# leftfield-geospatial/homonim

Measured on AMD Instinct MI355X. Metric: Mpixels*bands/s fit+apply (5x5 gain-offset, float32), higher is better.
Workload: dtype f32 in/out, f64 window sums; 1 GPU; synthetic float32 4-band 16384x16384 src/ref resident in HBM per GPU, Model.gain-offset, kernel 5x5, r2_inpaint_thresh 0.25, fused fit+apply (BASELINE.json configs[2]); bands=4, height=16384, width=16384, nodata_variant=0, parallelism=1 rank(s) x 1 GPU, one raster per rank, no collective

## Files before the change

### homonim_amd/csrc/hk_api.hip

```cpp
#include <hip/hip_runtime.h>

#include <algorithm>
#include <atomic>
#include <cfloat>
#include <cctype>
#include <cmath>
#include <condition_variable>
#include <cstdarg>
#include <cstdio>
#include <cstdlib>
#include <cstring>
#include <map>
#include <mutex>
#include <new>
#include <optional>
#include <vector>

#include "../../include/homonim_hk.h"
#include "../../include/homonim_hk_devtools.h"
#include "hk_kernels.h"

#include <dlfcn.h>
#include <hsa/hsa.h>
#include <hsa/hsa_ext_amd.h>
// ... 204 lines not shown
    size_t norm_ws_bytes = 0;
    void* aux = nullptr;
    size_t aux_bytes = 0;
    double* comm_xchg = nullptr;
    size_t comm_xchg_bytes = 0;
    unsigned long long* fail_host = nullptr;
    static constexpr size_t PIN_NORM = 64, PIN_SUMS = 128, PIN_NORM_IN = 192, PIN_WORD = 256, PIN_STATS = 512, PIN_COUNTS = 1024, PIN_BYTES = 16384;
    template <class T> T* pin(size_t off) const { return reinterpret_cast<T*>(reinterpret_cast<char*>(fail_host) + off); }
    static constexpr int STAGE_N = 4;
    struct StageOut {
        char* h_dst = nullptr;
        size_t h_pitch = 0, row_bytes = 0, c_pitch = 0;
        size_t rows = 0;
    };
    char* stage = nullptr;
    size_t stage_chunk = 0;
    hipEvent_t stage_ev[STAGE_N] = {nullptr, nullptr, nullptr, nullptr};
    int stage_state[STAGE_N] = {0, 0, 0, 0};
    StageOut stage_out[STAGE_N];
    int stage_next = 0;
    static constexpr int TBL_RING = 4;
    void* tbl_host[TBL_RING] = {nullptr, nullptr, nullptr, nullptr};
    void* tbl_dev[TBL_RING] = {nullptr, nullptr, nullptr, nullptr};
    size_t tbl_bytes[TBL_RING] = {0, 0, 0, 0};
    hipEvent_t tbl_ev[TBL_RING] = {nullptr, nullptr, nullptr, nullptr};
    int tbl_next = 0;
    unsigned* open_rows = nullptr;
    size_t open_rows_bytes = 0;
    bool direct_pending = false;
    bool busy = false;
    int dev_inflight = 0;
    bool dev_touched = false;
};

constexpr int64_t ROW_ALIGN = 64;

struct LaunchPolicy {
    int xcd_remap = 16;
    int force_general = 0;
    std::optional<int> use_ring;
    int wave_slots = 256 * 12;
    std::optional<int> seg_big, seg_tail;
};

}

struct hk_ctx {
    int device = 0;
    std::vector<Slot> slots;
    std::mutex mu;
    std::condition_variable cv;
    LaunchPolicy launch;
    std::atomic<int> expect_r2_failures{0};
    ncclComm_t comm = nullptr;
    int comm_rank = 0, comm_world = 0;
    std::mutex comm_mu;
    Slot xfer;
    std::mutex xfer_mu;
};

struct hk_event {
    hipEvent_t ev;
};

namespace {

void stage_abandon(Slot& s);

struct SlotLease {
    hk_ctx* ctx;
    int idx;
    SlotLease(hk_ctx* c) : ctx(c), idx(-1) {
        bool drain = false;
        {
            std::unique_lock<std::mutex> lk(ctx->mu);
            ctx->cv.wait(lk, [&] {
                int any = -1;
                for (size_t i = 0; i < ctx->slots.size(); ++i) {
                    if (ctx->slots[i].busy || ctx->slots[i].dev_inflight > 0) continue;
                    if (!ctx->slots[i].dev_touched) {
                        idx = (int)i;
                        return true;
                    }
                    if (any < 0) any = (int)i;
                }
                idx = any;
                return any >= 0;
            });
            ctx->slots[idx].busy = true;
            drain = ctx->slots[idx].dev_touched;
            ctx->slots[idx].dev_touched = false;
        }
        if (drain) (void)hipStreamSynchronize(ctx->slots[idx].stream);
    }
    ~SlotLease() {
        stage_abandon(ctx->slots[idx]);
        {
            std::lock_guard<std::mutex> lk(ctx->mu);
            ctx->slots[idx].busy = false;
        }
        ctx->cv.notify_all();
    }
    Slot& slot() { return ctx->slots[idx]; }
};

struct DevEnter {
// ... 469 lines not shown
    a.seg_rows = uniform < a.height ? uniform : a.height;
    a.seg_rows_tail = a.seg_rows;
    a.n_segs = (a.height + a.seg_rows - 1) / a.seg_rows;
    a.n_segs_big = a.n_segs;
    const long long per_row_band = (long long)a.n_strips * a.n_bands;
    if (seg_rows <= 0 && per_row_band * a.n_segs >= seg.two_size_from) {
        const int big = seg.big, tail = seg.tail;
        long long tail_rows = (long long)(seg.tail_waves / (double)per_row_band * big);
        tail_rows = (tail_rows + tail - 1) / tail * tail;
        if (big > 0 && tail > 0 && tail_rows < a.height - big) {
            const int n_big = (int)((a.height - tail_rows) / big);
            const int rest = a.height - n_big * big;
            a.seg_rows = big;
            a.seg_rows_tail = tail;
            a.n_segs_big = n_big;
            a.n_segs = n_big + (rest + tail - 1) / tail;
        }
    }
    a.total_units = a.n_strips * a.n_segs * a.n_bands;
    if (a.lds_pad < 0) a.lds_pad = lds_pad_of((long long)a.height * a.width * a.n_bands);
}

static int ensure_inpaint_scratch(Slot& sl, size_t plane, int height, long long stride) {
    return grow_slot_buf(sl, sl.aux, sl.aux_bytes, plane + hk::inpaint_workspace_bytes(height, stride));
}

static bool cert_list_eligible(const hk::FitArgs& a, const hk_fit_desc* desc) {
    return desc->model == HK_MODEL_GAIN_OFFSET && a.has_thresh && a.fail_count && !a.r2 && !a.gain && !a.flag && !a.offset_in &&
           !a.jobs && (a.use_ring == 1 || a.use_ring == 2) && (long long)desc->kh * desc->kw <= 65535;
}

static int launch_fit(hk_ctx* ctx, Slot& sl, hk::FitArgs& a, const hk_fit_desc* desc, bool r2) {
    a.cert_only = 0, a.open_rows = nullptr, a.list_mode = 0;
    if (!cert_list_eligible(a, desc)) {
        HK_HIP(hk::launch_fit_apply(a, desc->model, r2, sl.stream));
        return HK_OK;
    }
    const size_t bytes = (size_t)a.n_bands * (size_t)a.n_strips * (size_t)((a.height + 31) / 32) * sizeof(unsigned);
    {
        std::lock_guard<std::mutex> lk(ctx->mu);
        const int rc = grow_slot_buf(sl, sl.open_rows, sl.open_rows_bytes, bytes);
        if (rc) return rc;
    }
    hk::FitArgs c = a;
    c.open_rows = sl.open_rows;
    HK_HIP(hipMemsetAsync(c.open_rows, 0, bytes, sl.stream));
    c.cert_only = 1;
    HK_HIP(hk::launch_fit_apply(c, desc->model, r2, sl.stream));
    c.cert_only = 0, c.list_mode = 1;
    HK_HIP(hk::launch_fit_apply(c, desc->model, r2, sl.stream));
    return HK_OK;
}

static int inpaint_band(Slot& sl, const hk::FitArgs& a, const hk_fit_desc* desc, bool r2, size_t plane,
                        unsigned long long n_fail, bool drop_params = false, float* pre_offset = nullptr,
                        const unsigned char* pre_flag = nullptr) {
    {
        const int rc = ensure_inpaint_scratch(sl, plane, a.height, a.stride);
        if (rc) return rc;
    }
    const hipStream_t stream = sl.stream;
    char* aux = static_cast<char*>(sl.aux);
    const float *pg = a.gain, *pr = a.r2;
    float* po = a.offset;
    const unsigned char* flags = nullptr;
    if (pre_offset && pre_flag) {
        po = pre_offset, flags = pre_flag;
    } else if (!pg || !po || !pr) {
        float* scratch_off = reinterpret_cast<float*>(aux);
        hk::FitArgs b = a;
        b.gain = nullptr, b.r2 = nullptr, b.offset = scratch_off, b.corr = nullptr, b.fail_count = nullptr;
        b.flag = hk::inpaint_flag_plane(aux + plane, a.height, a.stride);
        b.cert_only = 0, b.open_rows = nullptr, b.list_mode = 0;
        HK_HIP(hk::launch_fit_apply(b, desc->model, r2, stream));
        po = scratch_off, flags = b.flag;
    }
    HK_HIP(hk::launch_inpaint_offsets(po, pg, pr, desc->r2_thresh, a.stride, a.height, a.width, aux + plane, stream, flags, n_fail));
    hk::FitArgs c = a;
    c.offset_in = po;
    c.flag_in = flags ? flags : hk::inpaint_flag_plane(aux + plane, a.height, a.stride);
    c.fail_count = nullptr;
    c.flag = nullptr;
    c.r2 = nullptr;
    c.cert_only = 0, c.open_rows = nullptr, c.list_mode = 0;
    if (drop_params) c.gain = c.offset = nullptr;
    HK_HIP(hk::launch_fit_apply(c, desc->model, false, stream));
    return HK_OK;
}

int job_fit_args(hk::FitArgs& a, const hk_ctx* ctx, const hk_fit_desc* desc, const hk_dev_job& job, int band = -1) {
    const int b = band < 0 ? 0 : band;
    const long long off = (long long)b * job.band_stride;
    auto plane = [off](float* p) { return p ? p + off : nullptr; };
    memset(&a, 0, sizeof(a));
    a.src = job.src + off, a.ref = job.ref + off;
    a.gain = plane(job.gain), a.offset = plane(job.offset), a.r2 = plane(job.r2), a.corr = plane(job.corr);
    a.norm = job.norm ? job.norm + 2 * b : nullptr;
    a.fail_count = job.fail_count ? reinterpret_cast<unsigned long long*>(job.fail_count) + b : nullptr;
    a.height = job.height, a.width = job.width, a.stride = job.stride;
    a.band_stride = band < 0 ? job.band_stride : 0;
    a.n_bands = band < 0 ? job.n_bands : 1;
    fill_args(a, desc, ctx->launch);
    fill_grid(a, job.seg_rows, ctx->launch);
    if (job.out_rows || job.out_cols) {
        if (a.has_thresh)
            return fail(HK_ERR_UNSUPPORTED, "a store window is not supported together with r2_inpaint_thresh (the in-painting "
                                            "needs the parameters of the whole block)");
        a.out_y0 = job.out_row0, a.out_y1 = job.out_row0 + job.out_rows;
        a.out_x0 = job.out_col0, a.out_x1 = job.out_col0 + job.out_cols;
    }
    return HK_OK;
}

hk::NormArgs norm_args(const hk_fit_desc* desc, const float* src, const float* ref, int height, int width, long long stride,
                       long long band_stride = 0, int n_bands = 1) {
    hk::NormArgs na;
    na.src = src, na.ref = ref, na.height = height, na.width = width, na.stride = stride;
    na.band_stride = band_stride, na.n_bands = n_bands;
    na.src_nd_mode = desc->src_nodata_mode, na.ref_nd_mode = desc->ref_nodata_mode;
    na.src_nodata = desc->src_nodata, na.ref_nodata = desc->ref_nodata;
    return na;
}

struct FitPending {
    hk::FitArgs a;
    bool scratch_params = false;
    bool active = false;
};

int fit_finish(hk_ctx* ctx, Slot& sl, const hk_fit_desc* desc, FitPending& p, unsigned long long n_fail, bool* requeued) {
    *requeued = false;
    if (!p.active) return HK_OK;
    hk::FitArgs& a = p.a;
    const bool r2 = needs_r2(desc);
    const size_t plane = (size_t)a.stride * a.height * sizeof(float);
    ctx->expect_r2_failures.store(n_fail > 0 ? 1 : 0);
    if (n_fail > 0) {
        const int rc = inpaint_band(sl, a, desc, r2, plane, n_fail, p.scratch_params, a.flag ? a.offset : nullptr, a.flag);
        if (rc) return rc;
        *requeued = true;
    }
    return HK_OK;
}

int fit_on_device(hk_ctx* ctx, Slot& sl, const hk_fit_desc* desc, const double* norm_in, float* d_src, float* d_ref,
                  int32_t height, int32_t width, int64_t stride, float* d_gain, float* d_off, float* d_r2, float* d_corr,
                  double* d_norm, unsigned long long* d_fail, void* d_norm_ws, FitPending* defer = nullptr,
                  const int* win = nullptr) {
    const bool blk = desc->model == HK_MODEL_GAIN_BLK_OFFSET;
    const bool r2 = needs_r2(desc);
    const size_t plane = (size_t)stride * height * sizeof(float);
    HK_HIP(hipMemsetAsync(d_fail, 0, sizeof(unsigned long long), sl.stream));
    if (blk) {
        if (norm_in) {
            memcpy(sl.pin<double>(Slot::PIN_NORM_IN), norm_in, 2 * sizeof(double));
            HK_HIP(hipMemcpyAsync(d_norm, sl.pin<double>(Slot::PIN_NORM_IN), 2 * sizeof(double), hipMemcpyHostToDevice, sl.stream));
        } else {
            HK_HIP(hk::launch_block_norm(norm_args(desc, d_src, d_ref, height, width, stride), d_norm_ws, d_norm, sl.stream));
        }
    }
    hk_dev_job job = {};
    job.src = d_src, job.ref = d_ref, job.gain = d_gain, job.offset = d_off, job.r2 = d_r2, job.corr = d_corr;
    job.norm = blk ? d_norm : nullptr;
    job.fail_count = reinterpret_cast<uint64_t*>(d_fail);
    job.n_bands = 1, job.height = height, job.width = width, job.stride = stride;
    if (win && !(desc->model == HK_MODEL_GAIN_OFFSET && desc->has_r2_thresh))
        job.out_row0 = win[0], job.out_rows = win[1] - win[0], job.out_col0 = win[2], job.out_cols = win[3] - win[2];
    FitPending local;
    FitPending& p = defer ? *defer : local;
    hk::FitArgs& a = p.a;
    int rc = job_fit_args(a, ctx, desc, job);
    if (rc) return rc;
    p.scratch_params = false;
    if (a.has_thresh && desc->model == HK_MODEL_GAIN_OFFSET && ctx->expect_r2_failures.load()) {
        rc = ensure_inpaint_scratch(sl, plane, height, stride);
        if (rc) return rc;
        char* aux = static_cast<char*>(sl.aux);
        a.flag = hk::inpaint_flag_plane(aux + plane, height, stride);
        if (!d_off) {
            a.offset = reinterpret_cast<float*>(aux);
            p.scratch_params = !d_gain && !d_r2;
        }
    }
    rc = launch_fit(ctx, sl, a, desc, r2);
    if (rc) return rc;
    p.active = a.has_thresh != 0;
    if (defer || !p.active) return HK_OK;

    HK_HIP(hipMemcpyAsync(sl.fail_host, d_fail, sizeof(unsigned long long), hipMemcpyDeviceToHost, sl.stream));
    HK_HIP(hipStreamSynchronize(sl.stream));
    bool requeued = false;
// ... 170 lines not shown
    int n = 0;
    if (hipGetDeviceCount(&n) != hipSuccess || n < 1)
        return fail(HK_ERR_NODEVICE, "no HIP device available (libhomonim_hk needs an MI355X / gfx950 GPU)");
    if (device_id < 0 || device_id >= n) return fail(HK_ERR_ARG, "device %d out of range [0, %d)", device_id, n);
    if (n_streams < 1) n_streams = 1;
    if (n_streams > 64) n_streams = 64;
    HK_HIP(hipSetDevice(device_id));
    hipDeviceProp_t prop;
    HK_HIP(hipGetDeviceProperties(&prop, device_id));
    if (strncmp(prop.gcnArchName, "gfx950", 6) != 0)
        return fail(HK_ERR_NODEVICE, "device %d is %s; this library is built for gfx950 only", device_id, prop.gcnArchName);
    hk_ctx* ctx = new (std::nothrow) hk_ctx();
    if (!ctx) return fail(HK_ERR_NOMEM, "out of host memory");
    ctx->device = device_id;
    ctx->slots.resize(n_streams);
    {
        auto env = [](const char* name) { const char* e = getenv(name); return e ? std::optional<int>(atoi(e)) : std::nullopt; };
        LaunchPolicy& lp = ctx->launch;
        if (const auto remap = env("HK_XCD_REMAP")) lp.xcd_remap = std::min(std::max(*remap, 0), 256);
        lp.force_general = env("HK_FORCE_GENERAL").value_or(0);
        lp.use_ring = env("HK_USE_RING");
        lp.wave_slots = env("HK_WAVE_SLOTS").value_or(lp.wave_slots);
        lp.seg_big = env("HK_SEG_BIG");
        lp.seg_tail = env("HK_SEG_TAIL");
    }
    for (auto& s : ctx->slots) {
        hipError_t e = hipStreamCreateWithFlags(&s.stream, hipStreamNonBlocking);
        if (e != hipSuccess) {
            hk_ctx_destroy(ctx);
            return fail(HK_ERR_HIP, "hipStreamCreate: %s", hipGetErrorString(e));
        }
        if (ensure_pin(s) != HK_OK) {
            hk_ctx_destroy(ctx);
            return HK_ERR_NOMEM;
        }
    }
    {
        hipError_t e = hipStreamCreateWithFlags(&ctx->xfer.stream, hipStreamNonBlocking);
        if (e != hipSuccess || ensure_pin(ctx->xfer) != HK_OK) {
            hk_ctx_destroy(ctx);
            return e != hipSuccess ? fail(HK_ERR_HIP, "hipStreamCreate: %s", hipGetErrorString(e)) : HK_ERR_NOMEM;
        }
    }
    register_gpu_fault_report();
    *out = ctx;
    return HK_OK;
}

int hk_ctx_destroy(hk_ctx* ctx) {
    if (!ctx) return HK_OK;
    (void)hipSetDevice(ctx->device);
    for (auto& s : ctx->slots) slot_release(s);
    slot_release(ctx->xfer);
    if (ctx->comm && rccl().ok) rccl().CommDestroy(ctx->comm);
    delete ctx;
    return HK_OK;
}

int hk_ctx_sync(hk_ctx* ctx) {
    if (!ctx) return fail(HK_ERR_ARG, "ctx is NULL");
    HK_ENTER(ctx);
    HK_HIP(hipDeviceSynchronize());
    return HK_OK;
}

int hk_block_norm(hk_ctx* ctx, const hk_fit_desc* desc, const float* src, int64_t src_stride, const float* ref,
                  int64_t ref_stride, int32_t height, int32_t width, double norm_out[2]) {
    if (!norm_out) return fail(HK_ERR_ARG, "norm_out is NULL");
    return run_host(ctx, desc, nullptr, src, src_stride, ref, ref_stride, height, width, nullptr, nullptr, 0, nullptr,
                    norm_out, nullptr, true);
}

int hk_fit(hk_ctx* ctx, const hk_fit_desc* desc, const float* src, int64_t src_stride, const float* ref,
           int64_t ref_stride, int32_t height, int32_t width, const double* norm_in, float* params_out,
           int32_t n_param_bands, double* norm_out, uint64_t* r2_fail_count) {
    if (!params_out) return fail(HK_ERR_ARG, "params_out is NULL");
    return run_host(ctx, desc, nullptr, src, src_stride, ref, ref_stride, height, width, norm_in, params_out,
                    n_param_bands, nullptr, norm_out, r2_fail_count, false);
}

int hk_fit_apply(hk_ctx* ctx, const hk_fit_desc* desc, const float* src, int64_t src_stride, const float* ref,
                 int64_t ref_stride, int32_t height, int32_t width, const double* norm_in, float* params_out,
                 int32_t n_param_bands, float* corr_out, double* norm_out, uint64_t* r2_fail_count) {
    if (!corr_out) return fail(HK_ERR_ARG, "corr_out is NULL");
    return run_host(ctx, desc, nullptr, src, src_stride, ref, ref_stride, height, width, norm_in, params_out,
                    n_param_bands, corr_out, norm_out, r2_fail_count, false);
}

int hk_fit_apply_io(hk_ctx* ctx, const hk_fit_desc* desc, const hk_io_desc* io, const void* src, int64_t src_stride,
                    const void* ref, int64_t ref_stride, int32_t height, int32_t width, const double* norm_in,
                    float* params_out, int32_t n_param_bands, void* corr_out, double* norm_out, uint64_t* r2_fail_count) {
    return run_host(ctx, desc, io, src, src_stride, ref, ref_stride, height, width, norm_in, params_out, n_param_bands,
                    corr_out, norm_out, r2_fail_count, false);
}

int hk_fit_apply_block(hk_ctx* ctx, const hk_fit_desc* desc, const hk_io_desc* io, const void* src, int64_t src_stride,
                       const void* ref, int64_t ref_stride, int32_t height, int32_t width, const double* norm_in,
                       float* params_out, int32_t n_param_bands, void* corr_out, const hk_out_window* window,
                       double* norm_out, uint64_t* r2_fail_count) {
    return run_host(ctx, desc, io, src, src_stride, ref, ref_stride, height, width, norm_in, params_out, n_param_bands,
                    corr_out, norm_out, r2_fail_count, false, window);
}

int hk_apply(hk_ctx* ctx, const float* src, int64_t src_stride, const float* params, int32_t height, int32_t width,
             float* out) {
    if (!ctx) return fail(HK_ERR_ARG, "ctx is NULL");
// ... 529 lines not shown
    HK_HIP(hipMemcpyAsync(host_counts, job->fail_count, bytes, hipMemcpyDeviceToHost, sl.stream));
    HK_HIP(hipMemsetAsync(job->fail_count, 0, bytes, sl.stream));
    HK_HIP(hipEventRecord(ready->ev, sl.stream));
    return HK_OK;
}

int hk_debug_stage_stamps(hk_ctx* ctx, uint64_t out[16], int32_t reset) {
    if (!ctx || !out) return fail(HK_ERR_ARG, "NULL argument");
    HK_ENTER(ctx);
    HK_HIP(hipDeviceSynchronize());
    unsigned long long tmp[16];
    HK_HIP(hk::read_stamps(tmp, reset != 0));
    for (int i = 0; i < 16; ++i) out[i] = tmp[i];
    return HK_OK;
}

int hk_r2_certificate_constants(float thresh, double* pass_below, double* fail_above, float* kappa, float* kappa_fail) {
    if (pass_below) *pass_below = r2_pass_scale(thresh);
    if (fail_above) *fail_above = r2_fail_above(thresh);
    if (kappa) *kappa = r2_fail_scale(thresh);
    if (kappa_fail) *kappa_fail = r2_failcert_scale(thresh);
    return HK_OK;
}

int hk_counts_pending(const uint64_t* counts, int32_t n_bands) {
    if (!counts) return 0;
    for (int32_t b = 0; b < n_bands; ++b)
        if (counts[b]) return 1;
    return 0;
}

int hk_event_sync(hk_ctx* ctx, hk_event* ev) {
    if (!ctx || !ev) return fail(HK_ERR_ARG, "NULL argument");
    HK_ENTER(ctx);
    HK_HIP(hipEventSynchronize(ev->ev));
    return HK_OK;
}

int hk_inpaint_dev_counts(hk_ctx* ctx, const hk_fit_desc* desc, const hk_dev_job* job, const uint64_t* counts,
                          uint64_t* n_fail_out) {
    int rc = validate_desc(desc);
    if (rc) return rc;
    rc = check_job(ctx, job);
    if (rc) return rc;
    DevEnter entered(ctx, job->stream);
    if (n_fail_out) *n_fail_out = 0;
    if (desc->model != HK_MODEL_GAIN_OFFSET || !desc->has_r2_thresh) return HK_OK;
    if (!counts) return fail(HK_ERR_ARG, "counts is NULL");
    HK_ENTER(ctx);
    Slot& sl = ctx->slots[job->stream];
    const bool r2 = needs_r2(desc);
    const size_t plane = (size_t)job->stride * job->height * sizeof(float);
    unsigned long long total = 0;
    for (int b = 0; b < job->n_bands; ++b) {
        unsigned long long n_fail = counts[b];
        if (n_fail == 0) continue;
        const long long off = (long long)b * job->band_stride;
        hk::FitArgs a;
        if ((rc = job_fit_args(a, ctx, desc, *job, b))) return rc;
        std::unique_lock<std::mutex> lk(ctx->mu);
        float* pre_off = nullptr;
        const unsigned char* pre_flag = nullptr;
        if (job->scratch) {
            pre_flag = job_scratch_flag(job) + off;
            pre_off = a.offset ? a.offset : job_scratch_offset(job) + off;
        }
        total += n_fail;
        rc = inpaint_band(sl, a, desc, r2, plane, n_fail, false, pre_off, pre_flag);
        if (rc) return rc;
    }
    if (n_fail_out) *n_fail_out = total;
    return HK_OK;
}

int hk_inpaint_dev(hk_ctx* ctx, const hk_fit_desc* desc, const hk_dev_job* job, uint64_t* n_fail_out) {
    int rc = validate_desc(desc);
    if (rc) return rc;
    rc = check_job(ctx, job);
    if (rc) return rc;
    DevEnter entered(ctx, job->stream);
    if (n_fail_out) *n_fail_out = 0;
    if (desc->model != HK_MODEL_GAIN_OFFSET || !desc->has_r2_thresh) return HK_OK;
    if (!job->fail_count) return fail(HK_ERR_ARG, "job->fail_count is NULL");
    if (job->n_bands > 1024) return fail(HK_ERR_ARG, "too many bands");
    HK_ENTER(ctx);
    Slot& sl = ctx->slots[job->stream];
    std::vector<uint64_t> counts((size_t)job->n_bands);
    uint64_t* const pinned = sl.pin<uint64_t>(Slot::PIN_COUNTS);
    HK_HIP(hipMemcpyAsync(pinned, job->fail_count, counts.size() * sizeof(uint64_t), hipMemcpyDeviceToHost, sl.stream));
    HK_HIP(hipStreamSynchronize(sl.stream));
    memcpy(counts.data(), pinned, counts.size() * sizeof(uint64_t));
    HK_HIP(hipMemsetAsync(job->fail_count, 0, counts.size() * sizeof(uint64_t), sl.stream));
    return hk_inpaint_dev_counts(ctx, desc, job, counts.data(), n_fail_out);
}

static int ensure_stream_ws(hk_ctx* ctx, Slot& sl, size_t need) {
    std::lock_guard<std::mutex> lk(ctx->mu);
    return grow_slot_buf(sl, sl.norm_ws, sl.norm_ws_bytes, need);
}

static int check_nodata_mode(int32_t mode) {
    return (mode == HK_NODATA_NONE || mode == HK_NODATA_NAN || mode == HK_NODATA_VALUE)
               ? HK_OK
               : fail(HK_ERR_ARG, "bad nodata mode %d", mode);
}

int hk_compare_sums_dev(hk_ctx* ctx, const hk_dev_job* job, int32_t src_nodata_mode, float src_nodata,
                        int32_t ref_nodata_mode, float ref_nodata, double* sums_dev) {
    int rc = check_job(ctx, job);
    if (rc) return rc;
    DevEnter entered(ctx, job->stream);
    if (!sums_dev) return fail(HK_ERR_ARG, "sums_dev is NULL");
    if ((rc = check_nodata_mode(src_nodata_mode)) || (rc = check_nodata_mode(ref_nodata_mode))) return rc;
    HK_ENTER(ctx);
    Slot& sl = ctx->slots[job->stream];
    rc = ensure_stream_ws(ctx, sl, hk::compare_workspace_bytes(job->n_bands));
    if (rc) return rc;
    hk::CompareArgs ca;
    memset(&ca, 0, sizeof(ca));
    ca.src = job->src, ca.ref = job->ref, ca.height = job->height, ca.width = job->width;
    ca.src_stride = ca.ref_stride = job->stride, ca.src_band_stride = ca.ref_band_stride = job->band_stride;
// ... 614 lines not shown
```

### homonim_amd/csrc/hk_fit_kernel.h

```cpp
#pragma once
#include "hk_kernels.h"

#include <type_traits>

namespace hk {

static __device__ unsigned long long hk_stamps[16];
#ifdef HK_STAMPS
#define HK_STAMP(k)                                                       \
    do {                                                                  \
        __builtin_amdgcn_sched_barrier(0);                                \
        const unsigned long long now_ = __builtin_amdgcn_s_memtime();     \
        st_acc[k] += now_ - st_prev;                                      \
        st_prev = now_;                                                   \
        __builtin_amdgcn_sched_barrier(0);                                \
    } while (0)
#else
#define HK_STAMP(k) do { } while (0)
#endif
static inline hipError_t read_stamps_tu(unsigned long long* acc16, bool reset) {
    unsigned long long v[16];
    hipError_t e = hipMemcpyFromSymbol(v, HIP_SYMBOL(hk_stamps), sizeof(v));
    if (e != hipSuccess) return e;
    for (int k = 0; k < 16; ++k) acc16[k] += v[k];
// ... 1219 lines not shown
                                } else if constexpr (BLK) {
                                    q = __dmul_rn((double)__fmul_rn(gp[i], gp[i]), HS2[i]);
                                    q = __dsub_rn(q, __dmul_rn((double)__fmul_rn(2.f, gp[i]), HP[i]));
                                    q = __dadd_rn(q, HR2[i]);
                                } else {
                                    q = __dmul_rn((double)__fmul_rn(g[i], g[i]), HS2[i]);
                                    q = __dsub_rn(q, (double)__fmul_rn(__fmul_rn(2.f, g[i]), Pf[i]));
                                    q = __dadd_rn(q, HR2[i]);
                                }
                                ssres[i] = __dmul_rn(q, (double)Nf[i]);
                            }
                            bool r2_ok[PX];
                            bool divide = !GO || a.r2 != nullptr;
                            if constexpr (GO) {
                                if (!divide) {
                                    bool unsure = false;
#pragma unroll
                                    for (int i = 0; i < PX; ++i) {
                                        const bool pos = sstot[i] > 0.0;
                                        const bool yes = pos & (ssres[i] < __dmul_rn(a.r2_pass_below, sstot[i]));
                                        const bool no = pos & (ssres[i] > __dmul_rn(a.r2_fail_above, sstot[i]));
                                        r2_ok[i] = yes;
                                        unsure |= out_lane & (bool)((mcu >> (8 * i)) & 1u) & !(yes | no);
                                    }
                                    divide = __any(unsure);
                                }
                            }
#pragma unroll
                            for (int i = 0; i < PX; ++i) {
                                if (divide) {
                                    r2v[i] = __fsub_rn(1.f, (float)__ddiv_rn(ssres[i], sstot[i]));
                                    r2_ok[i] = r2v[i] > a.r2_thresh;
                                }
                                if constexpr (GO) {
                                    const bool m = (mcu >> (8 * i)) & 1u;
                                    if (!(r2_ok[i] && (g[i] > 0.f))) passed &= ~(0xffu << (8 * i));
                                    const bool failing = count_fails && m && !(r2_ok[i] && (g[i] > 0.f));
                                    if (failing && out_lane) ++nfail;
                                    if (failing && inpaint_pass && out_lane) {
                                        const float oin = a.offset_in[out_base + (long long)y * a.stride + x + i];
                                        o[i] = oin;
                                        g[i] = __fdiv_rn(__fsub_rn(Rf[i], __fmul_rn(Nf[i], oin)), Sf[i]);
                                    }
                                }
                            }
                        }
                    }
                }

                if constexpr (GO && !R2) {
                    if (a.offset_in != nullptr) {
                        const long long q = out_base + (long long)y * a.stride + (lane_in ? x : 0);
                        const float4 oin4 = *reinterpret_cast<const float4*>(a.offset_in + q);
                        const unsigned fl = *reinterpret_cast<const unsigned*>(a.flag_in + q);
                        const float oin[PX] = {oin4.x, oin4.y, oin4.z, oin4.w};
#pragma unroll
                        for (int i = 0; i < PX; ++i) {
                            const bool failing = ((mcu >> (8 * i)) & 1u) && !((fl >> (8 * i)) & 0xffu);
                            if (failing) {
                                o[i] = oin[i];
                                g[i] = __fdiv_rn(__fsub_rn(Rf[i], __fmul_rn(Nf[i], oin[i])), Sf[i]);
                            }
                        }
                    }
                }

#pragma unroll
                for (int j = 0; j < PX / 2; ++j) {
                    const f2 c2 = HK_P2(g, j) * HK_P2(sc, j) + HK_P2(o, j);
                    c[2 * j] = c2.x, c[2 * j + 1] = c2.y;
                }
                if constexpr (!DENSE) {
#pragma unroll
                    for (int i = 0; i < PX; ++i) c[i] = ((mcu >> (8 * i)) & 1u) ? c[i] : qnan();
                }
                auto masked4 = [&](const float (&v)[PX]) {
                    float4 r4 = make_float4(v[0], v[1], v[2], v[3]);
                    if constexpr (!DENSE) {
                        r4.x = (mcu & 0x00000001u) ? r4.x : qnan();
                        r4.y = (mcu & 0x00000100u) ? r4.y : qnan();
                        r4.z = (mcu & 0x00010000u) ? r4.z : qnan();
                        r4.w = (mcu & 0x01000000u) ? r4.w : qnan();
                    }
                    return r4;
                };

                if (out_lane) {
                    const long long row_off = out_base + (long long)y * a.stride;
                    auto at = [&](float* plane) {
                        if constexpr (SB) return row_address(plane + row_off) + xbytes;
                        else return reinterpret_cast<float4*>(reinterpret_cast<char*>(plane + row_off) + xbytes);
                    };
                    if (a.corr && !((HK_ABLATE & 8) && c[0] != 123.456f)) store4_nt(at(a.corr), make_float4(c[0], c[1], c[2], c[3]));
                    if constexpr (!CERT_ONLY) {
                        if (a.gain) store4_nt(at(a.gain), masked4(g));
                    }
                    if (a.offset) store4_nt(at(a.offset), masked4(o));
                    if constexpr (!CERT_ONLY) {
                        if (R2 && a.r2) store4_nt(at(a.r2), masked4(r2v));
                    }
                    if constexpr (GO && R2 && !CERT_ONLY) {
                        if (a.flag) *reinterpret_cast<unsigned*>(a.flag + row_off + (xbytes >> 2)) = passed | ((~mcu & 0x01010101u) << 1);
                    }
                }
            };
            bool skip_row = false;
            if constexpr (LIST)
                skip_row = ((a.open_rows[(size_t)(band * a.n_strips + strip) * (size_t)((H + 31) >> 5) + (size_t)(y >> 5)] >> (y & 31)) & 1u) == 0u;
            if (skip_row) {
            } else if constexpr (UNIFORM_N) {
                if (n_uniform) pointwise(std::true_type{});
                else pointwise(std::false_type{});
            } else {
                pointwise(std::false_type{});
            }
            HK_STAMP(4);
        }

        if (++slot == ring_mod) slot = 0;
        if (++slot_c == ring_mod) slot_c = 0;
        if (++slot2 == rh + 1) slot2 = 0;
        if (++slot_r >= rh) slot_r = 0;
    }
#ifdef HK_STAMPS
    if (lane == 0) {
        for (int k = 0; k < 6; ++k) atomicAdd(&hk_stamps[k], st_acc[k]);
        atomicAdd(&hk_stamps[15], st_iters);
        atomicAdd(&hk_stamps[14], 1ull);
    }
#endif

    if constexpr (GO && R2) {
        if (a.fail_count != nullptr && a.has_thresh) {
#pragma unroll
            for (int d = WAVE / 2; d > 0; d >>= 1) nfail += __shfl_xor(nfail, d);
            if (lane == 0 && nfail) atomicAdd(a.fail_count + band, (unsigned long long)nfail);

        }
    }
}

template <int MODEL, bool R2, int RW, bool DENSE, int RING, bool CERT_ONLY, int WPB, bool BATCH = false>
__global__ void __launch_bounds__(WAVE * WPB, (fit_min_waves<MODEL, R2, RW, DENSE, RING, CERT_ONLY>()))
fit_apply_kernel(const FitArgs a_in) {
    extern __shared__ float4 lds4[];

    const int lane = threadIdx.x & (WAVE - 1), wave_in_wg = (WPB == 1 && fit_scalar_bases<MODEL, R2, RW, DENSE, RING, CERT_ONLY>()) ? 0 : threadIdx.x >> 6;
    int group = blockIdx.x;
    if (a_in.xcd_remap) {
        const int g = a_in.xcd_remap / WPB > 0 ? a_in.xcd_remap / WPB : 1, slot = blockIdx.x >> 3;
        group = ((slot / g) * 8 + (blockIdx.x & 7)) * g + slot % g;
    }
    [[maybe_unused]] FitArgs a_job;
    if constexpr (BATCH) {
        constexpr int FG = WPB > 1 ? 1 : 0;
// ... 242 lines not shown
```

### homonim_amd/csrc/hk_inpaint.hip

```cpp
#include "hk_kernels.h"

#include <stdlib.h>

#define HK_SQ(v) __mul24((v), (v))

#include <type_traits>

namespace hk {


__global__ void __launch_bounds__(256) inpaint_flag_kernel(const float* __restrict__ gain, const float* __restrict__ r2,
                                                           float thresh, long long stride, int height, int width,
                                                           unsigned char* __restrict__ flag) {
    const int x = blockIdx.x * blockDim.x + threadIdx.x;
    if (x >= width) return;
    for (int y = blockIdx.y; y < height; y += gridDim.y) {
        const long long i = (long long)y * stride + x;
        flag[i] = ((r2[i] > thresh) && (gain[i] > 0.f)) ? 1 : 0;
    }
}

constexpr unsigned NONE_B = 0xffu;
constexpr unsigned NONE_SQ = 0x7fffu;
constexpr int WORD_ROWS = 64;

__global__ void __launch_bounds__(256) inpaint_bits_kernel(const unsigned char* __restrict__ flag, long long stride, int height,
                                                           int width, unsigned long long* __restrict__ bits,
                                                           unsigned long long* __restrict__ tbits) {
    const int x = (blockIdx.x * blockDim.x + threadIdx.x) * 4;
    if (x >= width) return;
    const int y0 = blockIdx.y * WORD_ROWS;
    unsigned lo[4] = {0, 0, 0, 0}, hi[4] = {0, 0, 0, 0}, tlo[4] = {0, 0, 0, 0}, thi[4] = {0, 0, 0, 0};
#pragma unroll
    for (int r = 0; r < 32; ++r) {
        const int ya = y0 + r, yb = y0 + 32 + r;
        const unsigned fa = *reinterpret_cast<const unsigned*>(flag + (long long)min(ya, height - 1) * stride + x);
        const unsigned fb = *reinterpret_cast<const unsigned*>(flag + (long long)min(yb, height - 1) * stride + x);
#pragma unroll
        for (int c = 0; c < 4; ++c) {
            lo[c] |= (unsigned)(((fa >> (8 * c)) & 1u) != 0 && ya < height) << r;
            hi[c] |= (unsigned)(((fb >> (8 * c)) & 1u) != 0 && yb < height) << r;
            tlo[c] |= (unsigned)(((fa >> (8 * c)) & 0xffu) == 0 && ya < height) << r;
            thi[c] |= (unsigned)(((fb >> (8 * c)) & 0xffu) == 0 && yb < height) << r;
        }
    }
#pragma unroll
    for (int c = 0; c < 4; ++c)
        if (x + c < width) {
            bits[(long long)blockIdx.y * stride + x + c] = ((unsigned long long)hi[c] << 32) | lo[c];
            tbits[(long long)blockIdx.y * stride + x + c] = ((unsigned long long)thi[c] << 32) | tlo[c];
        }
}

__global__ void __launch_bounds__(256) inpaint_table_kernel(const unsigned long long* __restrict__ bits, long long stride,
                                                            int height, int width, int max_dist,
                                                            unsigned* __restrict__ tb) {
    const int x = (blockIdx.x * blockDim.x + threadIdx.x) * 2;
    if (x >= width) return;
    const int wb = blockIdx.y, n_words = (height + WORD_ROWS - 1) / WORD_ROWS;
    const int y0 = wb * WORD_ROWS, rows = min(WORD_ROWS, height - y0);
    unsigned long long wm2[2], wm1[2], w0[2], wp1[2], wp2[2];
#pragma unroll
    for (int c = 0; c < 2; ++c) {
        auto word = [&](int w) { return (w >= 0 && w < n_words) ? bits[(long long)w * stride + x + c] : 0ull; };
        wm2[c] = word(wb - 2), wm1[c] = word(wb - 1), w0[c] = word(wb), wp1[c] = word(wb + 1), wp2[c] = word(wb + 2);
    }
    constexpr int BIG = 1 << 20;
    unsigned upk[2][WORD_ROWS / 4];
    int dseed[2];
#pragma unroll
    for (int c = 0; c < 2; ++c) {
        int u = wm1[c] ? __clzll((long long)wm1[c]) : (wm2[c] ? 64 + __clzll((long long)wm2[c]) : BIG);
#pragma unroll
        for (int q = 0; q < WORD_ROWS / 4; ++q) {
            unsigned pk = 0;
#pragma unroll
            for (int k = 0; k < 4; ++k) {
                const int bb = 4 * q + k;
                u = ((w0[c] >> bb) & 1ull) ? 0 : min(u + 1, BIG);
                pk |= (unsigned)(u <= max_dist ? u : (int)NONE_B) << (8 * k);
            }
            upk[c][q] = pk;
        }
        dseed[c] = wp1[c] ? 1 + (__ffsll((long long)wp1[c]) - 1) : (wp2[c] ? 65 + (__ffsll((long long)wp2[c]) - 1) : BIG);
    }
    int d[2] = {dseed[0], dseed[1]};
#pragma unroll
    for (int bb = WORD_ROWS - 1; bb >= 0; --bb) {
        unsigned e[2];
#pragma unroll
        for (int c = 0; c < 2; ++c) {
            if (bb < WORD_ROWS - 1) d[c] = ((w0[c] >> (bb + 1)) & 1ull) ? 1 : min(d[c] + 1, BIG);
            const unsigned ub = (upk[c][bb >> 2] >> (8 * (bb & 3))) & 0xffu;
            const unsigned usq = ub == NONE_B ? NONE_SQ : (unsigned)HK_SQ((int)ub);
            const unsigned dsq = d[c] <= max_dist + 1 ? (unsigned)HK_SQ(d[c]) : NONE_SQ;
            e[c] = (dsq << 16) | usq;
// ... 326 lines not shown
                (unsigned char)(slow_rows[wv][lane >> 2] >> (8 * (lane & 3)));
    }
}

#ifndef HK_FILL_TILE_WAVES
#define HK_FILL_TILE_WAVES 8
#endif
template <int ROWS>
__global__ void __launch_bounds__(256, (ROWS <= 32 ? HK_FILL_TILE_WAVES : 5))
inpaint_fill_general_kernel(float* plane, const unsigned long long* __restrict__ bits, long long stride, int height, int width,
                            const unsigned* __restrict__ tb, const unsigned* __restrict__ tie, const double* __restrict__ wtab) {
    static_assert(ROWS == 16 || ROWS == 32 || ROWS == 64, "tiles divide the 64-row words of the bit planes");
    __shared__ unsigned short lst[256 / WAVE][ROWS * WAVE];
    const int tid = threadIdx.x, lane = tid & (WAVE - 1), wv = tid / WAVE;
    const int x0 = blockIdx.x * blockDim.x + wv * WAVE, x_own = x0 + lane;
    const unsigned long long lt = (1ull << lane) - 1ull;
    const int max_dist = FILL_MAX_DIST;
    const bool interior = x0 - max_dist - 12 >= 0 && x0 + WAVE - 1 + max_dist + 12 < width;
    const int n_tiles = (height + ROWS - 1) / ROWS;
    for (int tile_k = blockIdx.y; tile_k < n_tiles; tile_k += gridDim.y) {
        const int y0 = (n_tiles - 1 - tile_k) * ROWS;
        unsigned long long tgt_rows = 0ull;
        if (x_own < width) {
            tgt_rows = bits[(long long)(y0 / WORD_ROWS) * stride + x_own] >> (y0 % WORD_ROWS);
            const int rows_in = min(ROWS, height - y0);
            tgt_rows &= rows_in >= 64 ? ~0ull : (1ull << rows_in) - 1ull;
        }
        if (__ballot(tgt_rows != 0ull) == 0ull) continue;
        int n = 0;
#pragma unroll 4
        for (int r = 0; r < ROWS; ++r) {
            const bool target = (tgt_rows >> r) & 1ull;
            const unsigned long long bal = __ballot(target);
            if (target) lst[wv][n + (int)__popcll(bal & lt)] = (unsigned short)((r << 6) | lane);
            n += (int)__popcll(bal);
        }
        __builtin_amdgcn_fence(__ATOMIC_ACQ_REL, "wavefront");
        for (int p = 0; p < n; p += WAVE) {
            if (p + lane < n) {
                const unsigned e = lst[wv][p + lane];
                const int x = x0 + (int)(e & 63u), y = y0 + (int)(e >> 6);
                const long long row = (long long)y * stride;
                const bool last_row = y == height - 1;
                const float v = interior ? fill_one<true>(x, y, row, plane, stride, width, max_dist, tb, tie, wtab, last_row)
                                         : fill_one<false>(x, y, row, plane, stride, width, max_dist, tb, tie, wtab, last_row);
                plane[row + x] = v;
            }
        }
    }
}

static size_t bit_words(int height, long long stride) { return (size_t)((height + WORD_ROWS - 1) / WORD_ROWS) * (size_t)stride; }
size_t inpaint_workspace_bytes(int height, long long stride) {
    return (size_t)height * stride * 5 + 1024 + TIE_N / 8 + 256 + WTAB_N * 8 + 256 + 3 * (bit_words(height, stride) * 8 + 256)
           + sizeof(FastTables) + 256;
}

unsigned char* inpaint_flag_plane(void* workspace, int height, long long stride) {
    return reinterpret_cast<unsigned char*>(static_cast<unsigned short*>(workspace) + 2 * (size_t)height * stride);
}

hipError_t launch_inpaint_offsets(float* offset, const float* gain, const float* r2, float thresh, long long stride,
                                  int height, int width, void* workspace, hipStream_t stream,
                                  const unsigned char* flag_ready, unsigned long long n_targets) {
    const size_t plane = (size_t)height * stride;
    unsigned* tb = static_cast<unsigned*>(workspace);
    unsigned char* ws_flag = inpaint_flag_plane(workspace, height, stride);
    const unsigned char* flag = flag_ready ? flag_ready : ws_flag;
    unsigned* tie = reinterpret_cast<unsigned*>(ws_flag + (plane + 255) / 256 * 256);
    double* wtab = reinterpret_cast<double*>(tie + (TIE_N / 32 + 64) / 64 * 64);
    HK_LAUNCH(tie_kernel, dim3((TIE_N / 32 + 255) / 256), dim3(256), 0, stream, tie, wtab);
    const int max_dist = FILL_MAX_DIST;
    static_assert(100 + 1 < (int)NONE_B, "the table's distance bytes");
    if (!flag_ready)
        HK_LAUNCH(inpaint_flag_kernel, dim3((width + 255) / 256, height < 1024 ? height : 1024), dim3(256), 0, stream,
                           gain, r2, thresh, stride, height, width, ws_flag);
    auto align256 = [](void* p) { return reinterpret_cast<void*>((reinterpret_cast<uintptr_t>(p) + 255) / 256 * 256); };
    unsigned long long* bits = static_cast<unsigned long long*>(align256(wtab + WTAB_N));
    unsigned long long* tbits = static_cast<unsigned long long*>(align256(bits + bit_words(height, stride)));
    unsigned long long* sbits = static_cast<unsigned long long*>(align256(tbits + bit_words(height, stride)));
    FastTables* ftab = static_cast<FastTables*>(align256(sbits + bit_words(height, stride)));
    HK_LAUNCH(fast_table_kernel, dim3((FTAB_N + 7 + 255) / 256), dim3(256), 0, stream, ftab);
    const dim3 gbits((width + 1023) / 1024, (height + WORD_ROWS - 1) / WORD_ROWS);
    HK_LAUNCH(inpaint_bits_kernel, gbits, dim3(256), 0, stream, flag, stride, height, width, bits, tbits);
    const dim3 gtable((width + 511) / 512, (height + WORD_ROWS - 1) / WORD_ROWS);
    HK_LAUNCH(inpaint_table_kernel, gtable, dim3(256), 0, stream, bits, stride, height, width, max_dist, tb);
    const bool by_column = (double)n_targets > 0.6 * (double)height * (double)width;
    const bool fast = stride < (1ll << 23);
    if (fast) {
        const int n_tiles8 = (height + 7) / 8, wgs_y = (n_tiles8 + 3) / 4;
        const dim3 gf((width + 255) / 256, wgs_y < 65535 ? wgs_y : 65535);
        if (by_column)
            HK_LAUNCH(inpaint_fill_fast_kernel<true>, gf, dim3(256), 0, stream, offset, tbits, sbits, stride, height, width, tb, ftab, 1);
        else
            HK_LAUNCH(inpaint_fill_fast_kernel<false>, gf, dim3(256), 0, stream, offset, tbits, sbits, stride, height, width, tb, ftab, 1);
    }
    const unsigned long long* todo = fast ? sbits : tbits;
    const int n_tiles = (height + 31) / 32;
    const dim3 gt((width + 255) / 256, n_tiles < 65535 ? n_tiles : 65535);
    HK_LAUNCH(inpaint_fill_general_kernel<32>, gt, dim3(256), 0, stream, offset, todo, stride, height, width, tb, tie, wtab);
    return hipGetLastError();
}

}
```

### homonim_amd/csrc/hk_kernels.h

```cpp
#pragma once
#include <hip/hip_runtime.h>
#include <stdint.h>
#include <string.h>

struct hk_warp_desc;

namespace hk {

constexpr int PX = 4;
constexpr int WAVE = 64;

struct BuildRecord {
    char name[88];
    unsigned long long launches;
    BuildRecord* next;
    explicit BuildRecord(const char* kernel_name);
    BuildRecord(int model, bool r2, int rw, bool dense, int ring, bool cert_only, int wpb, bool batch);
    BuildRecord(const char* kernel_name, int model, bool r2, int rw, bool dense, int ring);
    void hit() { __atomic_fetch_add(&launches, 1ull, __ATOMIC_RELAXED); }
};
template <typename Tag>
struct SiteRecord {
    static BuildRecord rec;
};
// ... 151 lines not shown
    int src_nd_mode, ref_nd_mode;
    float src_nodata, ref_nodata;
    int vec_ok;
};
size_t compare_workspace_bytes(int n_bands);
hipError_t launch_compare_sums(const CompareArgs& a, void* workspace, double* sums_out, hipStream_t stream);

constexpr int PARAM_STATS_N = 10;
struct ParamStatsArgs {
    const float* planes;
    int height, width;
    long long stride;
    long long band_stride;
    int n_bands;
    int nd_mode;
    float nodata;
    double thresh;
    int vec_ok;
};
size_t param_stats_workspace_bytes(int n_bands);
hipError_t launch_param_stats(const ParamStatsArgs& a, void* workspace, double* stats_out, hipStream_t stream);

constexpr int OVERVIEW_PASS_LEVELS = 6;
struct OverviewArgs {
    const void* src;
    int height, width;
    long long stride, band_stride;
    int nd_mode;
    int n_levels;
    double nodata;
    void* out[OVERVIEW_PASS_LEVELS];
    long long out_stride[OVERVIEW_PASS_LEVELS], out_band_stride[OVERVIEW_PASS_LEVELS];
    int vec_ok, out_vec_ok;
};
hipError_t launch_overviews(int dtype, const void* src, int height, int width, long long stride, long long band_stride,
                            int n_bands, int nd_mode, double nodata, int n_levels, void* const* out, const long long* out_stride,
                            const long long* out_band_stride, hipStream_t stream);

hipError_t launch_synth_fill(float* src, float* ref, int n_bands, int height, int width, long long stride,
                             long long band_stride, unsigned long long seed, int nodata_variant, hipStream_t stream);

hipError_t launch_cast_in(int dtype, const void* in, long long in_stride, float* out, long long out_stride, int height,
                          int width, hipStream_t stream);
hipError_t launch_cast_out(int dtype, const float* in, long long in_stride, void* out, long long out_stride, int height,
                           int width, int has_nodata, double nodata, hipStream_t stream);
inline int dtype_size(int dtype) { const int sz[7] = {4, 1, 2, 2, 4, 4, 8}; return dtype >= 0 && dtype < 7 ? sz[dtype] : 0; }

hipError_t launch_partial_mask(const float* in, int nd_mode, float nodata, const float* params, int n_bands,
                               long long band_stride, const float* src, int height, int width, long long stride, int kh,
                               int kw, unsigned short* rowcnt_ws, float* params_out, float* corr_out,
                               unsigned char* mask_out, hipStream_t stream);

size_t inpaint_workspace_bytes(int height, long long stride);
unsigned char* inpaint_flag_plane(void* workspace, int height, long long stride);
hipError_t launch_inpaint_offsets(float* offset, const float* gain, const float* r2, float thresh, long long stride,
                                  int height, int width, void* workspace, hipStream_t stream,
                                  const unsigned char* flag_ready = nullptr, unsigned long long n_targets = 0);

hipError_t launch_resample(int mode, const float* src, long long src_stride, long long src_band_stride, int sh, int sw,
                           int n_bands, int nd_mode, float nodata, double kx, double ox, double ky, double oy, float* dst,
                           long long dst_stride, long long dst_band_stride, int dh, int dw, float dst_fill,
                           hipStream_t stream);

hipError_t launch_warp_coords(const hk_warp_desc* desc, double off_row, double off_col, double* x, double* y, long long stride,
                              int h, int w, hipStream_t stream, const char** why);
hipError_t launch_warp_resample(int mode, const hk_warp_desc* desc, const float* src, long long src_stride,
                                long long src_band_stride, int sh, int sw, int n_bands, int nd_mode, float nodata, double kx,
                                double ky, float* dst, long long dst_stride, long long dst_band_stride, int dh, int dw,
                                float dst_fill, hipStream_t stream, const char** why);

size_t upsample_apply_workspace_bytes(int height);
hipError_t launch_upsample_apply(int mode, const float* src, long long src_stride, int nd_mode, float nodata,
                                 const float* gain, const float* offset, long long par_stride, int ph, int pw,
                                 const float* keep, long long keep_stride, float* out, long long out_stride, int height,
                                 int width, double kx, double ox, double ky, double oy, void* workspace, hipStream_t stream);
hipError_t launch_valid_plane(const float* in, long long in_stride, int nd_mode, float nodata, float* out,
                              long long out_stride, int height, int width, hipStream_t stream);
hipError_t launch_apply_space(const float* src, long long src_stride, int nd_mode, float nodata, const float* gain,
                              const float* offset, long long par_stride, const float* keep, float* out,
                              long long out_stride, int height, int width, hipStream_t stream);

hipError_t launch_stream_probe(const void* a, const void* b, void* out, size_t n_bytes, hipStream_t stream);

hipError_t launch_checksum(const float* plane, long long stride, int height, int width, unsigned long long* out_dev, hipStream_t stream);

hipError_t launch_selftest(int* result_dev, hipStream_t stream);

}
```

Before: 356,700 Mpixels*bands/s.

## Pack inpaint flags to one byte per four pixels and cache lookup tables

```diff
diff --git a/homonim_amd/csrc/hk_api.hip b/homonim_amd/csrc/hk_api.hip
--- a/homonim_amd/csrc/hk_api.hip
+++ b/homonim_amd/csrc/hk_api.hip
@@ -280,6 +280,7 @@
     std::condition_variable cv;
     LaunchPolicy launch;
     std::atomic<int> expect_r2_failures{0};
+    void* inpaint_tables = nullptr;
     ncclComm_t comm = nullptr;
     int comm_rank = 0, comm_world = 0;
     std::mutex comm_mu;
@@ -855,9 +856,27 @@
     return HK_OK;
 }
 
-static int inpaint_band(Slot& sl, const hk::FitArgs& a, const hk_fit_desc* desc, bool r2, size_t plane,
-                        unsigned long long n_fail, bool drop_params = false, float* pre_offset = nullptr,
-                        const unsigned char* pre_flag = nullptr) {
+static int inpaint_tables(hk_ctx* ctx, hipStream_t stream, const void** tables) {
+    std::lock_guard<std::mutex> lk(ctx->mu);
+    if (!ctx->inpaint_tables) {
+        void* p = nullptr;
+        if (dev_malloc(&p, hk::inpaint_tables_bytes()) != hipSuccess)
+            return fail(HK_ERR_NOMEM, "hipMalloc(%zu) failed", hk::inpaint_tables_bytes());
+        hipError_t e = hk::launch_inpaint_tables(p, stream);
+        if (e == hipSuccess) e = hipStreamSynchronize(stream);
+        if (e != hipSuccess) {
+            (void)dev_free(p);
+            return fail(HK_ERR_HIP, "building the in-painting tables failed: %s", hipGetErrorString(e));
+        }
+        ctx->inpaint_tables = p;
+    }
+    *tables = ctx->inpaint_tables;
+    return HK_OK;
+}
+
+static int inpaint_search(Slot& sl, const void* tables, const hk::FitArgs& a, const hk_fit_desc* desc, bool r2, size_t plane,
+                          unsigned long long n_fail, float* pre_offset, const unsigned char* pre_flag, float** po_out,
+                          const unsigned char** flags_out) {
     {
         const int rc = ensure_inpaint_scratch(sl, plane, a.height, a.stride);
         if (rc) return rc;
@@ -878,17 +897,33 @@
         HK_HIP(hk::launch_fit_apply(b, desc->model, r2, stream));
         po = scratch_off, flags = b.flag;
     }
-    HK_HIP(hk::launch_inpaint_offsets(po, pg, pr, desc->r2_thresh, a.stride, a.height, a.width, aux + plane, stream, flags, n_fail));
+    HK_HIP(hk::launch_inpaint_offsets(po, pg, pr, desc->r2_thresh, a.stride, a.height, a.width, aux + plane, tables, stream, flags, n_fail));
+    *po_out = po;
+    *flags_out = flags ? flags : hk::inpaint_flag_plane(aux + plane, a.height, a.stride);
+    return HK_OK;
+}
+
+static int inpaint_close(Slot& sl, const hk::FitArgs& a, const hk_fit_desc* desc, const float* po, const unsigned char* flags,
+                         bool drop_params) {
     hk::FitArgs c = a;
     c.offset_in = po;
-    c.flag_in = flags ? flags : hk::inpaint_flag_plane(aux + plane, a.height, a.stride);
+    c.flag_in = flags;
     c.fail_count = nullptr;
     c.flag = nullptr;
     c.r2 = nullptr;
     c.cert_only = 0, c.open_rows = nullptr, c.list_mode = 0;
     if (drop_params) c.gain = c.offset = nullptr;
-    HK_HIP(hk::launch_fit_apply(c, desc->model, false, stream));
-    return HK_OK;
+    HK_HIP(hk::launch_fit_apply(c, desc->model, false, sl.stream));
+    return HK_OK;
+}
+
+static int inpaint_band(Slot& sl, const void* tables, const hk::FitArgs& a, const hk_fit_desc* desc, bool r2, size_t plane,
+                        unsigned long long n_fail, bool drop_params = false, float* pre_offset = nullptr,
+                        const unsigned char* pre_flag = nullptr) {
+    float* po = nullptr;
+    const unsigned char* flags = nullptr;
+    const int rc = inpaint_search(sl, tables, a, desc, r2, plane, n_fail, pre_offset, pre_flag, &po, &flags);
+    return rc ? rc : inpaint_close(sl, a, desc, po, flags, drop_params);
 }
 
 int job_fit_args(hk::FitArgs& a, const hk_ctx* ctx, const hk_fit_desc* desc, const hk_dev_job& job, int band = -1) {
@@ -939,7 +974,10 @@
     const size_t plane = (size_t)a.stride * a.height * sizeof(float);
     ctx->expect_r2_failures.store(n_fail > 0 ? 1 : 0);
     if (n_fail > 0) {
-        const int rc = inpaint_band(sl, a, desc, r2, plane, n_fail, p.scratch_params, a.flag ? a.offset : nullptr, a.flag);
+        const void* tables = nullptr;
+        int rc = inpaint_tables(ctx, sl.stream, &tables);
+        if (rc) return rc;
+        rc = inpaint_band(sl, tables, a, desc, r2, plane, n_fail, p.scratch_params, a.flag ? a.offset : nullptr, a.flag);
         if (rc) return rc;
         *requeued = true;
     }
@@ -1216,6 +1254,7 @@
     (void)hipSetDevice(ctx->device);
     for (auto& s : ctx->slots) slot_release(s);
     slot_release(ctx->xfer);
+    if (ctx->inpaint_tables) (void)dev_free(ctx->inpaint_tables);
     if (ctx->comm && rccl().ok) rccl().CommDestroy(ctx->comm);
     delete ctx;
     return HK_OK;
@@ -1851,8 +1890,12 @@
     const bool r2 = needs_r2(desc);
     const size_t plane = (size_t)job->stride * job->height * sizeof(float);
     unsigned long long total = 0;
+    for (int b = 0; b < job->n_bands; ++b) total += counts[b];
+    if (total == 0) return HK_OK;
+    const void* tables = nullptr;
+    if ((rc = inpaint_tables(ctx, sl.stream, &tables))) return rc;
     for (int b = 0; b < job->n_bands; ++b) {
-        unsigned long long n_fail = counts[b];
+        const unsigned long long n_fail = counts[b];
         if (n_fail == 0) continue;
         const long long off = (long long)b * job->band_stride;
         hk::FitArgs a;
@@ -1861,11 +1904,10 @@
         float* pre_off = nullptr;
         const unsigned char* pre_flag = nullptr;
         if (job->scratch) {
-            pre_flag = job_scratch_flag(job) + off;
+            pre_flag = job_scratch_flag(job) + off / 4;
             pre_off = a.offset ? a.offset : job_scratch_offset(job) + off;
         }
-        total += n_fail;
-        rc = inpaint_band(sl, a, desc, r2, plane, n_fail, false, pre_off, pre_flag);
+        rc = inpaint_band(sl, tables, a, desc, r2, plane, n_fail, false, pre_off, pre_flag);
         if (rc) return rc;
     }
     if (n_fail_out) *n_fail_out = total;
diff --git a/homonim_amd/csrc/hk_fit_kernel.h b/homonim_amd/csrc/hk_fit_kernel.h
--- a/homonim_amd/csrc/hk_fit_kernel.h
+++ b/homonim_amd/csrc/hk_fit_kernel.h
@@ -1295,11 +1295,13 @@
                     if (a.offset_in != nullptr) {
                         const long long q = out_base + (long long)y * a.stride + (lane_in ? x : 0);
                         const float4 oin4 = *reinterpret_cast<const float4*>(a.offset_in + q);
-                        const unsigned fl = *reinterpret_cast<const unsigned*>(a.flag_in + q);
+                        typedef __attribute__((address_space(1))) const unsigned char gflag;
+                        const unsigned fl = *(gflag*)(row_address(a.flag_in + ((out_base + (long long)y * a.stride) >> 2)) + (xq >> 4));
                         const float oin[PX] = {oin4.x, oin4.y, oin4.z, oin4.w};
+                        const unsigned tfail = mcu & ((fl >> 4) * 0x00204081u);
 #pragma unroll
                         for (int i = 0; i < PX; ++i) {
-                            const bool failing = ((mcu >> (8 * i)) & 1u) && !((fl >> (8 * i)) & 0xffu);
+                            const bool failing = (tfail >> (8 * i)) & 1u;
                             if (failing) {
                                 o[i] = oin[i];
                                 g[i] = __fdiv_rn(__fsub_rn(Rf[i], __fmul_rn(Nf[i], oin[i])), Sf[i]);
@@ -1343,7 +1345,12 @@
                         if (R2 && a.r2) store4_nt(at(a.r2), masked4(r2v));
                     }
                     if constexpr (GO && R2 && !CERT_ONLY) {
-                        if (a.flag) *reinterpret_cast<unsigned*>(a.flag + row_off + (xbytes >> 2)) = passed | ((~mcu & 0x01010101u) << 1);
+                        if (a.flag) {
+                            unsigned fq = (passed & 0x01010101u) | (((mcu ^ passed) & 0x01010101u) << 4);
+                            fq |= fq >> 7;
+                            fq |= fq >> 14;
+                            a.flag[(row_off >> 2) + (xbytes >> 4)] = (unsigned char)fq;
+                        }
                     }
                 }
             };
diff --git a/homonim_amd/csrc/hk_inpaint.hip b/homonim_amd/csrc/hk_inpaint.hip
--- a/homonim_amd/csrc/hk_inpaint.hip
+++ b/homonim_amd/csrc/hk_inpaint.hip
@@ -12,11 +12,16 @@
 __global__ void __launch_bounds__(256) inpaint_flag_kernel(const float* __restrict__ gain, const float* __restrict__ r2,
                                                            float thresh, long long stride, int height, int width,
                                                            unsigned char* __restrict__ flag) {
-    const int x = blockIdx.x * blockDim.x + threadIdx.x;
+    const int x = (blockIdx.x * blockDim.x + threadIdx.x) * 4;
     if (x >= width) return;
+    const unsigned inside = x + 3 < width ? 0xfu : (1u << (width - x)) - 1u;
     for (int y = blockIdx.y; y < height; y += gridDim.y) {
         const long long i = (long long)y * stride + x;
-        flag[i] = ((r2[i] > thresh) && (gain[i] > 0.f)) ? 1 : 0;
+        unsigned src = 0u;
+#pragma unroll
+        for (int c = 0; c < 4; ++c)
+            if ((inside >> c) & 1u) src |= (unsigned)((r2[i + c] > thresh) && (gain[i + c] > 0.f)) << c;
+        flag[i >> 2] = (unsigned char)(src | ((~src & inside) << 4));
     }
 }
 
@@ -34,14 +39,15 @@
 #pragma unroll
     for (int r = 0; r < 32; ++r) {
         const int ya = y0 + r, yb = y0 + 32 + r;
-        const unsigned fa = *reinterpret_cast<const unsigned*>(flag + (long long)min(ya, height - 1) * stride + x);
-        const unsigned fb = *reinterpret_cast<const unsigned*>(flag + (long long)min(yb, height - 1) * stride + x);
+        unsigned fa = flag[((long long)min(ya, height - 1) * stride + x) >> 2];
+        unsigned fb = flag[((long long)min(yb, height - 1) * stride + x) >> 2];
+        fa = ya < height ? fa : 0u, fb = yb < height ? fb : 0u;
 #pragma unroll
         for (int c = 0; c < 4; ++c) {
-            lo[c] |= (unsigned)(((fa >> (8 * c)) & 1u) != 0 && ya < height) << r;
-            hi[c] |= (unsigned)(((fb >> (8 * c)) & 1u) != 0 && yb < height) << r;
-            tlo[c] |= (unsigned)(((fa >> (8 * c)) & 0xffu) == 0 && ya < height) << r;
-            thi[c] |= (unsigned)(((fb >> (8 * c)) & 0xffu) == 0 && yb < height) << r;
+            lo[c] |= ((fa >> c) & 1u) << r;
+            hi[c] |= ((fb >> c) & 1u) << r;
+            tlo[c] |= ((fa >> (4 + c)) & 1u) << r;
+            thi[c] |= ((fb >> (4 + c)) & 1u) << r;
         }
     }
 #pragma unroll
@@ -474,35 +480,44 @@
 
 static size_t bit_words(int height, long long stride) { return (size_t)((height + WORD_ROWS - 1) / WORD_ROWS) * (size_t)stride; }
 size_t inpaint_workspace_bytes(int height, long long stride) {
-    return (size_t)height * stride * 5 + 1024 + TIE_N / 8 + 256 + WTAB_N * 8 + 256 + 3 * (bit_words(height, stride) * 8 + 256)
-           + sizeof(FastTables) + 256;
+    return (size_t)height * stride * 5 + 1024 + 3 * (bit_words(height, stride) * 8 + 256);
 }
 
 unsigned char* inpaint_flag_plane(void* workspace, int height, long long stride) {
     return reinterpret_cast<unsigned char*>(static_cast<unsigned short*>(workspace) + 2 * (size_t)height * stride);
 }
 
+static constexpr size_t TABLES_TIE = 0, TABLES_WTAB = (TIE_N / 8 + 255) / 256 * 256,
+                        TABLES_FAST = TABLES_WTAB + ((size_t)WTAB_N * 8 + 255) / 256 * 256;
+size_t inpaint_tables_bytes() { return TABLES_FAST + sizeof(FastTables); }
+hipError_t launch_inpaint_tables(void* tables, hipStream_t stream) {
+    char* t = static_cast<char*>(tables);
+    HK_LAUNCH(tie_kernel, dim3((TIE_N / 32 + 255) / 256), dim3(256), 0, stream, reinterpret_cast<unsigned*>(t + TABLES_TIE),
+              reinterpret_cast<double*>(t + TABLES_WTAB));
+    HK_LAUNCH(fast_table_kernel, dim3((FTAB_N + 7 + 255) / 256), dim3(256), 0, stream, reinterpret_cast<FastTables*>(t + TABLES_FAST));
+    return hipGetLastError();
+}
+
 hipError_t launch_inpaint_offsets(float* offset, const float* gain, const float* r2, float thresh, long long stride,
-                                  int height, int width, void* workspace, hipStream_t stream,
+                                  int height, int width, void* workspace, const void* tables, hipStream_t stream,
                                   const unsigned char* flag_ready, unsigned long long n_targets) {
     const size_t plane = (size_t)height * stride;
     unsigned* tb = static_cast<unsigned*>(workspace);
     unsigned char* ws_flag = inpaint_flag_plane(workspace, height, stride);
     const unsigned char* flag = flag_ready ? flag_ready : ws_flag;
-    unsigned* tie = reinterpret_cast<unsigned*>(ws_flag + (plane + 255) / 256 * 256);
-    double* wtab = reinterpret_cast<double*>(tie + (TIE_N / 32 + 64) / 64 * 64);
-    HK_LAUNCH(tie_kernel, dim3((TIE_N / 32 + 255) / 256), dim3(256), 0, stream, tie, wtab);
+    const char* t = static_cast<const char*>(tables);
+    const unsigned* tie = reinterpret_cast<const unsigned*>(t + TABLES_TIE);
+    const double* wtab = reinterpret_cast<const double*>(t + TABLES_WTAB);
+    const FastTables* ftab = reinterpret_cast<const FastTables*>(t + TABLES_FAST);
     const int max_dist = FILL_MAX_DIST;
     static_assert(100 + 1 < (int)NONE_B, "the table's distance bytes");
     if (!flag_ready)
-        HK_LAUNCH(inpaint_flag_kernel, dim3((width + 255) / 256, height < 1024 ? height : 1024), dim3(256), 0, stream,
+        HK_LAUNCH(inpaint_flag_kernel, dim3((width + 1023) / 1024, height < 1024 ? height : 1024), dim3(256), 0, stream,
                            gain, r2, thresh, stride, height, width, ws_flag);
     auto align256 = [](void* p) { return reinterpret_cast<void*>((reinterpret_cast<uintptr_t>(p) + 255) / 256 * 256); };
-    unsigned long long* bits = static_cast<unsigned long long*>(align256(wtab + WTAB_N));
+    unsigned long long* bits = static_cast<unsigned long long*>(align256(ws_flag + plane));
     unsigned long long* tbits = static_cast<unsigned long long*>(align256(bits + bit_words(height, stride)));
     unsigned long long* sbits = static_cast<unsigned long long*>(align256(tbits + bit_words(height, stride)));
-    FastTables* ftab = static_cast<FastTables*>(align256(sbits + bit_words(height, stride)));
-    HK_LAUNCH(fast_table_kernel, dim3((FTAB_N + 7 + 255) / 256), dim3(256), 0, stream, ftab);
     const dim3 gbits((width + 1023) / 1024, (height + WORD_ROWS - 1) / WORD_ROWS);
     HK_LAUNCH(inpaint_bits_kernel, gbits, dim3(256), 0, stream, flag, stride, height, width, bits, tbits);
     const dim3 gtable((width + 511) / 512, (height + WORD_ROWS - 1) / WORD_ROWS);
diff --git a/homonim_amd/csrc/hk_kernels.h b/homonim_amd/csrc/hk_kernels.h
--- a/homonim_amd/csrc/hk_kernels.h
+++ b/homonim_amd/csrc/hk_kernels.h
@@ -227,9 +227,11 @@
                                unsigned char* mask_out, hipStream_t stream);
 
 size_t inpaint_workspace_bytes(int height, long long stride);
+size_t inpaint_tables_bytes();
+hipError_t launch_inpaint_tables(void* tables, hipStream_t stream);
 unsigned char* inpaint_flag_plane(void* workspace, int height, long long stride);
 hipError_t launch_inpaint_offsets(float* offset, const float* gain, const float* r2, float thresh, long long stride,
-                                  int height, int width, void* workspace, hipStream_t stream,
+                                  int height, int width, void* workspace, const void* tables, hipStream_t stream,
                                   const unsigned char* flag_ready = nullptr, unsigned long long n_targets = 0);
 
 hipError_t launch_resample(int mode, const float* src, long long src_stride, long long src_band_stride, int sh, int sw,
```

New measurement: 357,500 Mpixels*bands/s (median of 4 runs). Within noise of the previous version (+0.2%).
